# ctu-vras/monoforce

Hardware: AMD Instinct MI355X
Metric: rollout-steps/sec (batch x horizon) on 256x256 terrain (higher is better)
Workload: dtype f32; 1 GPU; c3: B=1024/GPU x T=500 x N=4 contact points, 256x256 grid (res 0.05 m), one shared terrain+friction map (the same on every rank), integrator=odeint-euler (reference default), forward+backward; BASE...; rollouts_per_gpu=1024, rollouts_total=1024, horizon=500, contact_points=4, parallelism=rollout-sharded x1

## Files before the change

monoforce_amd/csrc/physics_loss.hip:

```cpp
#include "mf_common.h"

namespace mf {

__device__ __forceinline__ void atomic_add_s(float* p, float v) { unsafeAtomicAdd(p, v); }
__device__ __forceinline__ void atomic_add_s(double* p, double v) { unsafeAtomicAdd(p, v); }

template <typename S>
__global__ void __launch_bounds__(256) physics_loss_fwd_kernel(const S* __restrict__ Xs, long long sb, long long st,
                                                              const S* __restrict__ Xgt, const S* __restrict__ gt_ts,
                                                              const int* __restrict__ nearest, int B, int T2, S gamma,
                                                              S* __restrict__ partial) {
  __shared__ S wave_sum[4];
  const int i = blockIdx.x * blockDim.x + threadIdx.x;
  S acc = (S)0;
  if (i < B * T2) {
    const int b = i / T2;
    const S w = (S)1 / ((S)1 + gamma * gt_ts[i]);
    const S* x = Xs + b * sb + (long long)nearest[i] * st;
    const S* g = Xgt + (size_t)i * 3;
#pragma unroll
    for (int c = 0; c < 3; ++c) { const S d = x[c] * w - g[c] * w; acc += d * d; }
  }
#pragma unroll
  for (int d = 32; d >= 1; d >>= 1) acc += __shfl_xor(acc, d, 64);
  if ((threadIdx.x & 63) == 0) wave_sum[threadIdx.x >> 6] = acc;
  __syncthreads();
  if (threadIdx.x == 0) partial[blockIdx.x] = (wave_sum[0] + wave_sum[1]) + (wave_sum[2] + wave_sum[3]);
}

template <typename S>
__global__ void __launch_bounds__(256) physics_loss_value_kernel(const S* __restrict__ Xs, long long sb, long long st,
                                                                const S* __restrict__ Xgt, const S* __restrict__ gt_ts,
                                                                const int* __restrict__ nearest, int B, int T2, S gamma,
                                                                S* __restrict__ partial, unsigned* __restrict__ ticket, S inv_count,
                                                                S* __restrict__ loss, S* __restrict__ zero_fill, long long zero_count) {
  __shared__ S wave_sum[4];
  __shared__ bool last;
  const int i = blockIdx.x * blockDim.x + threadIdx.x;
  {
    const long long head = min(zero_count, (long long)(((16u - (unsigned)((uintptr_t)zero_fill & 15u)) & 15u) / sizeof(S)));
    const long long n16 = (zero_count - head) * (long long)sizeof(S) / 16, tail0 = head + n16 * (16 / (long long)sizeof(S));
    int4* z16 = reinterpret_cast<int4*>(zero_fill + head);
    for (long long k = i; k < n16; k += (long long)gridDim.x * blockDim.x) z16[k] = make_int4(0, 0, 0, 0);
    if (i < head) zero_fill[i] = (S)0;
    if (tail0 + i < zero_count) zero_fill[tail0 + i] = (S)0;
  }
  S acc = (S)0;
  if (i < B * T2) {
    const int k = i, b = i / T2;
    const S w = (S)1 / ((S)1 + gamma * gt_ts[k]);
    const S* x = Xs + b * sb + (long long)nearest[k] * st;
    const S* g = Xgt + (size_t)k * 3;
#pragma unroll
    for (int c = 0; c < 3; ++c) { const S d = x[c] * w - g[c] * w; acc += d * d; }
  }
#pragma unroll
  for (int d = 32; d >= 1; d >>= 1) acc += __shfl_xor(acc, d, 64);
  if ((threadIdx.x & 63) == 0) wave_sum[threadIdx.x >> 6] = acc;
  __syncthreads();
  if (threadIdx.x == 0) {
    partial[blockIdx.x] = (wave_sum[0] + wave_sum[1]) + (wave_sum[2] + wave_sum[3]);
    __threadfence();
    last = atomicAdd(ticket, 1u) == gridDim.x - 1;
  }
  __syncthreads();
  if (!last) return;
  __threadfence();
  S tot = (S)0;
  for (unsigned k = threadIdx.x; k < gridDim.x; k += 256) tot += __builtin_nontemporal_load(partial + k);
#pragma unroll
  for (int d = 32; d >= 1; d >>= 1) tot += __shfl_xor(tot, d, 64);
  if ((threadIdx.x & 63) == 0) wave_sum[threadIdx.x >> 6] = tot;
  __syncthreads();
  if (threadIdx.x == 0) {
    loss[0] = ((wave_sum[0] + wave_sum[1]) + (wave_sum[2] + wave_sum[3])) * inv_count;
    *ticket = 0u;
  }
}

template <typename S>
__global__ void __launch_bounds__(256) reduce_grad_copies_kernel(S* __restrict__ pool, int copies, long long n, S* __restrict__ out) {
  const long long i = (long long)blockIdx.x * blockDim.x + threadIdx.x;
  if (i >= n) return;
  S* p = pool + (long long)blockIdx.y * copies * n + i;
  S acc = (S)0;
  for (int c = 0; c < copies; ++c) { acc += p[(long long)c * n]; p[(long long)c * n] = (S)0; }
  out[(long long)blockIdx.y * n + i] = acc;
}

template <typename S>
__global__ void __launch_bounds__(256) physics_loss_bwd_kernel(const S* __restrict__ Xs, long long sb, long long st,
                                                              const S* __restrict__ Xgt, const S* __restrict__ gt_ts,
                                                              const int* __restrict__ nearest, int B, int T2, S gamma,
                                                              const S* __restrict__ gloss, S inv_count, S* __restrict__ gXs) {
  const int t = blockIdx.x * blockDim.x + threadIdx.x;
  if (t >= B * T2) return;
  const bool jm = sb < st;
  const int b = jm ? t % B : t / T2, j = jm ? t / B : t % T2;
  const int i = b * T2 + j;
  const S scale = (S)2 * gloss[0] * inv_count;
  const S w = (S)1 / ((S)1 + gamma * gt_ts[i]);
  const int nr = nearest[i];
  const long long o = b * sb + (long long)nr * st;
  const S* g = Xgt + (size_t)i * 3;
  bool shared = false;
  for (int k = 0; k < T2; ++k) shared |= (k != j) & (nearest[b * T2 + k] == nr);
#pragma unroll
  for (int c = 0; c < 3; ++c) {
    const S v = scale * w * (Xs[o + c] * w - g[c] * w);
    if (shared) atomic_add_s(gXs + o + c, v); else gXs[o + c] = v;
  }
}

template <typename S>
static int loss_fwd(const MfLossDesc* d, const S* Xs, const S* Xgt, const S* gt_ts, const int* nearest, S* partial, hipStream_t st) {
  MF_REQUIRE(d && Xs && Xgt && gt_ts && nearest && partial, MF_ERR_INVALID, "physics_loss_fwd: null argument");
  MF_REQUIRE(d->B > 0 && d->T1 > 0 && d->T2 > 0, MF_ERR_INVALID, "physics_loss_fwd: B, T1, T2 must be positive");
  hipLaunchKernelGGL((physics_loss_fwd_kernel<S>), dim3((d->B * d->T2 + 255) / 256), dim3(256), 0, st, Xs, (long long)d->x_stride_b,
                     (long long)d->x_stride_t, Xgt, gt_ts, nearest, d->B, d->T2, (S)d->gamma, partial);
  hipError_t e = hipGetLastError();
  MF_REQUIRE(e == hipSuccess, MF_ERR_LAUNCH, std::string("physics_loss_fwd launch: ") + hipGetErrorString(e));
  return MF_OK;
}

template <typename S>
static int loss_value(const MfLossDesc* d, const S* Xs, const S* Xgt, const S* gt_ts, const int* nearest, S* partial, unsigned* ticket,
                      S* loss, S* zero_fill, long long zero_count, hipStream_t st) {
  MF_REQUIRE(d && Xs && Xgt && gt_ts && nearest && partial && ticket && loss, MF_ERR_INVALID, "physics_loss_value: null argument");
  MF_REQUIRE(d->B > 0 && d->T1 > 0 && d->T2 > 0, MF_ERR_INVALID, "physics_loss_value: B, T1, T2 must be positive");
  MF_REQUIRE(zero_count >= 0 && (zero_fill || zero_count == 0), MF_ERR_INVALID, "physics_loss_value: zero_count without zero_fill");
  const double count = (double)d->B * d->T2 * 3;
  hipLaunchKernelGGL((physics_loss_value_kernel<S>), dim3((d->B * d->T2 + 255) / 256), dim3(256), 0, st, Xs, (long long)d->x_stride_b,
                     (long long)d->x_stride_t, Xgt, gt_ts, nearest, d->B, d->T2, (S)d->gamma, partial, ticket, (S)(1.0 / count), loss, zero_fill, zero_count);
  hipError_t e = hipGetLastError();
  MF_REQUIRE(e == hipSuccess, MF_ERR_LAUNCH, std::string("physics_loss_value launch: ") + hipGetErrorString(e));
  return MF_OK;
}

template <typename S>
static int reduce_copies(S* pool, int n_maps, int copies, long long n, S* out, hipStream_t st) {
  MF_REQUIRE(pool && out, MF_ERR_INVALID, "reduce_grad_copies: null argument");
  MF_REQUIRE(n_maps > 0 && n_maps < 65536 && copies > 0 && n > 0, MF_ERR_INVALID, "reduce_grad_copies: n_maps, copies, n must be positive");
  hipLaunchKernelGGL((reduce_grad_copies_kernel<S>), dim3((unsigned)((n + 255) / 256), (unsigned)n_maps), dim3(256), 0, st, pool, copies, n, out);
  hipError_t e = hipGetLastError();
  MF_REQUIRE(e == hipSuccess, MF_ERR_LAUNCH, std::string("reduce_grad_copies launch: ") + hipGetErrorString(e));
  return MF_OK;
}

template <typename S>
static int loss_bwd(const MfLossDesc* d, const S* Xs, const S* Xgt, const S* gt_ts, const int* nearest, const S* gloss, S* gXs,
                    hipStream_t st) {
  MF_REQUIRE(d && Xs && Xgt && gt_ts && nearest && gloss && gXs, MF_ERR_INVALID, "physics_loss_bwd: null argument");
  MF_REQUIRE(d->B > 0 && d->T1 > 0 && d->T2 > 0, MF_ERR_INVALID, "physics_loss_bwd: B, T1, T2 must be positive");
  const double count = (double)d->B * d->T2 * 3;
  hipLaunchKernelGGL((physics_loss_bwd_kernel<S>), dim3((d->B * d->T2 + 255) / 256), dim3(256), 0, st, Xs, (long long)d->x_stride_b,
                     (long long)d->x_stride_t, Xgt, gt_ts, nearest, d->B, d->T2, (S)d->gamma, gloss, (S)(1.0 / count), gXs);
  hipError_t e = hipGetLastError();
  MF_REQUIRE(e == hipSuccess, MF_ERR_LAUNCH, std::string("physics_loss_bwd launch: ") + hipGetErrorString(e));
  return MF_OK;
}

}

namespace mf {
template <typename S>
__global__ void __launch_bounds__(256) nearest_steps_kernel(const S* __restrict__ pred_ts, long long pred_sb, const S* __restrict__ gt_ts, long long gt_sb,
                                                           int B, int T1, int T2, int* __restrict__ out) {
  const int i = blockIdx.x * blockDim.x + threadIdx.x;
  if (i >= B * T2) return;
  const int b = i / T2, j = i - b * T2;
  const S g = gt_ts[b * gt_sb + j];
  const S* p = pred_ts + b * pred_sb;
  S best = (S)INFINITY;
  int arg = 0;
  bool any = false;
  int t = 0;
  for (; t + 8 <= T1; t += 8) {
    S v[8];
#pragma unroll
    for (int k = 0; k < 8; ++k) v[k] = p[t + k];
#pragma unroll
    for (int k = 0; k < 8; ++k) {
      const S d = fabs(v[k] - g);
      if (d < best || (!any && d == d)) { best = d; arg = t + k; any = true; }
    }
  }
  for (; t < T1; ++t) {
    const S d = fabs(p[t] - g);
    if (d < best || (!any && d == d)) { best = d; arg = t; any = true; }
  }
  out[i] = arg;
}
template <typename S>
static int nearest_steps(int B, int T1, int T2, const S* pred_ts, long long pred_sb, const S* gt_ts, long long gt_sb, int32_t* out, hipStream_t st) {
  MF_REQUIRE(B > 0 && T1 > 0 && T2 > 0 && pred_ts && gt_ts && out && pred_sb >= 0 && gt_sb >= 0, MF_ERR_INVALID, "nearest_steps: bad argument");
  const long long n = (long long)B * T2;
  MF_REQUIRE(n < (1ll << 31), MF_ERR_UNSUPPORTED, "nearest_steps: B * T2 must be below 2^31");
  hipLaunchKernelGGL((nearest_steps_kernel<S>), dim3((unsigned)((n + 255) / 256)), dim3(256), 0, st, pred_ts, pred_sb, gt_ts, gt_sb, B, T1, T2, out);
  hipError_t e = hipGetLastError();
  MF_REQUIRE(e == hipSuccess, MF_ERR_LAUNCH, std::string("nearest_steps launch: ") + hipGetErrorString(e));
  return MF_OK;
}
}
extern "C" int mf_nearest_steps_f32(int32_t B, int32_t T1, int32_t T2, const float* pred_ts, long long pred_stride_b, const float* gt_ts, long long gt_stride_b,
                                    int32_t* nearest, void* s) { return mf::nearest_steps<float>(B, T1, T2, pred_ts, pred_stride_b, gt_ts, gt_stride_b, nearest, (hipStream_t)s); }
extern "C" int mf_nearest_steps_f64(int32_t B, int32_t T1, int32_t T2, const double* pred_ts, long long pred_stride_b, const double* gt_ts, long long gt_stride_b,
                                    int32_t* nearest, void* s) { return mf::nearest_steps<double>(B, T1, T2, pred_ts, pred_stride_b, gt_ts, gt_stride_b, nearest, (hipStream_t)s); }
extern "C" int mf_physics_loss_fwd_f32(const MfLossDesc* d, const float* Xs, const float* Xgt, const float* gt_ts, const int32_t* nearest,
                                       float* partial, void* s) { return mf::loss_fwd<float>(d, Xs, Xgt, gt_ts, nearest, partial, (hipStream_t)s); }
extern "C" int mf_physics_loss_fwd_f64(const MfLossDesc* d, const double* Xs, const double* Xgt, const double* gt_ts, const int32_t* nearest,
                                       double* partial, void* s) { return mf::loss_fwd<double>(d, Xs, Xgt, gt_ts, nearest, partial, (hipStream_t)s); }
extern "C" int mf_physics_loss_bwd_f32(const MfLossDesc* d, const float* Xs, const float* Xgt, const float* gt_ts, const int32_t* nearest,
                                       const float* gloss, float* gXs, void* s) { return mf::loss_bwd<float>(d, Xs, Xgt, gt_ts, nearest, gloss, gXs, (hipStream_t)s); }
extern "C" int mf_physics_loss_bwd_f64(const MfLossDesc* d, const double* Xs, const double* Xgt, const double* gt_ts, const int32_t* nearest,
                                       const double* gloss, double* gXs, void* s) { return mf::loss_bwd<double>(d, Xs, Xgt, gt_ts, nearest, gloss, gXs, (hipStream_t)s); }
extern "C" int mf_physics_loss_value_f32(const MfLossDesc* d, const float* Xs, const float* Xgt, const float* gt_ts, const int32_t* nearest,
                                         float* partial, uint32_t* ticket, float* loss, float* zero_fill, long long zero_count, void* s) { return mf::loss_value<float>(d, Xs, Xgt, gt_ts, nearest, partial, ticket, loss, zero_fill, zero_count, (hipStream_t)s); }
extern "C" int mf_physics_loss_value_f64(const MfLossDesc* d, const double* Xs, const double* Xgt, const double* gt_ts, const int32_t* nearest,
                                         double* partial, uint32_t* ticket, double* loss, double* zero_fill, long long zero_count, void* s) { return mf::loss_value<double>(d, Xs, Xgt, gt_ts, nearest, partial, ticket, loss, zero_fill, zero_count, (hipStream_t)s); }
extern "C" int mf_reduce_grad_copies_f32(float* pool, int n_maps, int copies, long long n, float* out, void* s) { return mf::reduce_copies<float>(pool, n_maps, copies, n, out, (hipStream_t)s); }
extern "C" int mf_reduce_grad_copies_f64(double* pool, int n_maps, int copies, long long n, double* out, void* s) { return mf::reduce_copies<double>(pool, n_maps, copies, n, out, (hipStream_t)s); }
```

monoforce_amd/csrc/rollout_bwd_cp_kernel.h:

```cpp
#pragma once
#include "rollout_bwd_kernel.h"
#include "rollout_cp_common.h"
#include <type_traits>

namespace mf {

#ifdef MF_STREAM_PROFILE
extern __device__ unsigned long long mf_stream_prof[32];
#define MF_PROF_T(v) const unsigned long long v = __builtin_readcyclecounter()
#define MF_PROF_RT(v) const unsigned long long v = __builtin_amdgcn_s_memrealtime()
#define MF_PROF_ACC(name) unsigned long long name = 0
#define MF_PROF_SUM(name, t0) name += __builtin_readcyclecounter() - (t0)
#define MF_PROF_OUT(slot, val) do { if (lane == 0) atomicAdd(&mf_stream_prof[slot], (unsigned long long)(val)); } while (0)
#define MF_PROF_ADD(slot, t0) MF_PROF_OUT(slot, __builtin_readcyclecounter() - (t0))
#define MF_PROF_MAX(slot, val) do { if (lane == 0) atomicMax(&mf_stream_prof[slot], (unsigned long long)(val)); } while (0)
#define MF_PROF_DRAIN() asm volatile("s_waitcnt vmcnt(0) lgkmcnt(0)" ::: "memory")
#else
#define MF_PROF_T(v)
#define MF_PROF_RT(v)
#define MF_PROF_ACC(name)
#define MF_PROF_SUM(name, t0)
#define MF_PROF_OUT(slot, val)
#define MF_PROF_ADD(slot, t0)
#define MF_PROF_MAX(slot, val)
// ... 928 lines not shown
          const S gzq = -gdh;
          const S dotn = dot3(gn, c.nrm);
          const S gg = (gn - dotn * c.nrm) * c.inlr;
          const S ggp = dpp<0x51>(gg);
          const S nz = mf_fma(gzq, c.wq, cgA * gg + cgB * ggp);
          const S nm = gmuq * c.wq;
          {
            const unsigned ni = (unsigned)c.idx;
            const bool same = !act | (ni == acc_idx);
            st_pending = !same;
            st_idx = acc_idx; st_z = acc_z; st_m = acc_m;
            acc_idx = act ? ni : acc_idx;
            acc_z = same ? acc_z + nz : nz;
            acc_m = same ? acc_m + nm : nm;
          }
          const S vq = gzq * c.zc + gmuq * c.mcv;
          const S gpx = dot4(vq, c.wsb), gpy = dot4(vq, c.wsa);
          const S gp = mask_or(mask_or(mask_or(zero, gpx, lane0), gpy, lane1), gdh, lane2);
          const S gvp1 = dpp<kRot1>(gvp), gvp2 = dpp<kRot2>(gvp);
          gr += gvp1 * c.w2 - gvp2 * c.w1;
          const S gw_p = c.r1 * gvp2 - c.r2 * gvp1;
          const S qa = gp + gr;
          lx += gp; lxd += gvp; lw += gw_p;
          lR0 = mf_fma(qa, P0, lR0); lR1 = mf_fma(qa, P1, lR1); lR2 = mf_fma(qa, P2, lR2);
          S gv = zero, gwc = zero;
          if constexpr (GCTRL) { gv = sum_points(gv_p); gwc = sum_points(gwc_p); }
          lR0 = mf_fma(-dot3(ge_p, c.e), c.eci, mf_fma(ge_p, c.il, lR0));
          gctrl_pending = __builtin_amdgcn_readfirstlane((unsigned)n * kC); gv_pending = gv; gwc_pending = gwc;
        };
        auto crunch = [&](int n, const Coef& c, const UpIn& up, Coef& c_next, UpIn& up_next, auto more, auto paired) {
          add_upstream_masked(up);
          if constexpr (decltype(paired)::value == 1) grab(c_next, up_next);
          else if constexpr (decltype(paired)::value == 2) { grab(c_next, up_next); release(); }
          else if constexpr (decltype(more)::value) take(c_next, up_next);
          flush_stash();
          if constexpr (GCTRL) bstore2(rGctrl, v_ctrl, gctrl_pending, gv_pending, gwc_pending);
#ifdef MF_STREAM_NO_VJP
          asm volatile("" :: "v"(c.R0), "v"(c.w1), "v"(c.f1), "v"(c.NnG), "v"(c.cmdv), "v"(c.csm), "v"(c.dcs), "v"(c.vp), "v"(c.zc), "v"(c.e));
#else
          chain(n, c, up);
#endif
        };
        using std::true_type;
        using std::false_type;
        Coef cA, cB;
        if (n_steps > 0) {
          take(cA, uA);
          MF_PROF_ADD(3, t_k0); MF_PROF_OUT(19, acc_wait);
          using single = std::integral_constant<int, 0>;
          for (; n >= 2; n -= 2) {
            ensure(2);
            crunch(n, cA, uA, cB, uB, true_type{}, std::integral_constant<int, 1>{});
            crunch(n - 1, cB, uB, cA, uA, true_type{}, std::integral_constant<int, 2>{});
          }
          if (n == 1) { crunch(1, cA, uA, cB, uB, true_type{}, single{}); crunch(0, cB, uB, cA, uA, false_type{}, single{}); }
          else crunch(0, cA, uA, cB, uB, false_type{}, single{});
        }
        MF_PROF_ADD(9, t_compute);
        MF_PROF_OUT(8, acc_wait);
#ifdef MF_STREAM_PROFILE
        MF_PROF_OUT(22, acc_wait_early); MF_PROF_OUT(23, n_waited); MF_PROF_OUT(24, acc_wait_late);
#endif
        MF_PROF_ADD(20, t_k0);
        MF_PROF_DRAIN();
        MF_PROF_T(t_sw);
        if (!a.skip_snap) {
          while (__builtin_amdgcn_readfirstlane(vflags[3]) == 0) __builtin_amdgcn_s_sleep(1);
          asm volatile("" ::: "memory");
          snap_idx = idx_of(snap_c[lane]); snap_wq = snap_c[64 + lane]; snap_dx = snap_c[128 + lane]; snap_dy = snap_c[192 + lane];
        }
        MF_PROF_DRAIN();
        MF_PROF_ADD(7, t_sw);
        uA = uZ; uB = uZ;
    } else {
      struct Raw { StateIn st; Saved sv; };
      Raw S_[3];
      Rec K_[3];
      UpIn U_[3];
      auto up_row = [&](int m) { return ODE ? max(m + 1, 0) : max(m, 0); };
      auto run = [&](auto rtag, int n) {
        constexpr int R = decltype(rtag)::value, R1 = (R + 1) % 3, R2 = (R + 2) % 3;
        add_upstream_state(U_[R]);
        gather_cells(S_[R1].sv);
#ifndef MF_SAVED_NO_STATE
        load_state(max(n - 3, 0), S_[R].st);
#endif
#ifndef MF_SAVED_NO_REC
        load_saved(max(n - 3, 0), S_[R].sv);
#endif
#ifndef MF_SAVED_NO_UP
        load_upstream(min(up_row(n - 2), a.T - 1), U_[R2]);
#endif
#ifndef MF_SAVED_NO_ATOMIC
        flush_stash();
#endif
        if constexpr (GCTRL) bstore2(rGctrl, v_ctrl, gctrl_pending, gv_pending, gwc_pending);
#ifndef MF_SAVED_NO_VJP
        vjp(n, K_[R], U_[R]);
#endif
#ifndef MF_SAVED_NO_VJP
        asm("" : "+v"(S_[R1].sv.zc), "+v"(S_[R1].sv.mc) : "v"(lR0));
#endif
#ifndef MF_SAVED_NO_REBUILD
        rebuild(S_[R1].st, S_[R1].sv, K_[R1]);
#endif
      };
      const int n0 = max(n, 0);
      load_state(n0, S_[0].st);
      load_saved(n0, S_[0].sv);
      load_upstream(min(up_row(n0), a.T - 1), U_[0]);
      load_state(max(n0 - 1, 0), S_[1].st);
      load_saved(max(n0 - 1, 0), S_[1].sv);
      load_upstream(min(up_row(n0 - 1), a.T - 1), U_[1]);
      load_state(max(n0 - 2, 0), S_[2].st);
      load_saved(max(n0 - 2, 0), S_[2].sv);
      gather_cells(S_[0].sv);
      rebuild(S_[0].st, S_[0].sv, K_[0]);
      __builtin_amdgcn_s_waitcnt(0);
      using std::integral_constant;
      int i = 0;
      for (; i + 2 < n_steps; i += 3) {
        run(integral_constant<int, 0>{}, n0 - i);
        run(integral_constant<int, 1>{}, n0 - i - 1);
        run(integral_constant<int, 2>{}, n0 - i - 2);
      }
      if (i < n_steps) run(integral_constant<int, 0>{}, n0 - i);
      if (i + 1 < n_steps) run(integral_constant<int, 1>{}, n0 - i - 1);
      {
        const int r0 = (n0 + 1) % 3;
        uA = r0 == 0 ? U_[0] : (r0 == 1 ? U_[1] : U_[2]);
        uB = uA;
      }
      n = -1;
    }
  } else {
  load_state(max(n, 0), sA);
  load_upstream(min(max(n, 0) + (ODE ? 1 : 0), a.T - 1), uA);
  load_state(max(n - 1, 0), sB);
  recompute_gather(sA, recA);
  recompute(recA);
  __builtin_amdgcn_s_waitcnt(0);
  for (; n >= 1; n -= 2) {
    body(n, recA, recB, sB, sA, uA, uB);
    body(n - 1, recB, recA, sA, sB, uB, uA);
  }
  if (n == 0) body(0, recA, recB, sB, sA, uA, uB);
  }
  MF_PROF_T(t_e0);
  UpIn up = (n_steps & 1) ? uB : uA;
  flush_stash();
  if constexpr (GCTRL) bstore2(rGctrl, v_ctrl, gctrl_pending, gv_pending, gwc_pending);
  if (act) emit(acc_idx, acc_z, acc_m);
  if constexpr (ODE) {
    if (n_steps == 0) load_upstream(0, up);
    add_upstream_state(up);
  }
  lx = sum_points(lx); lxd = sum_points(lxd); lw = sum_points(lw);
  lR0 = sum_points(lR0); lR1 = sum_points(lR1); lR2 = sum_points(lR2);
  MF_PROF_DRAIN();
  MF_PROF_ADD(10, t_e0);
  MF_PROF_T(t_s0);

  S gx0 = lx;
  if (!a.skip_snap) {
    if constexpr (!STREAM) snap_cell(snap_idx, snap_wq, snap_dx, snap_dy);
    const S g = dpp<kB2>(lx) / (S)a.N;
    if (act) atomic_add(at32(gzmap, goff + (unsigned)snap_idx), g * snap_wq);
    const S gpx = snap_dx * g * a.inv_res, gpy = snap_dy * g * a.inv_res;
    S gpxy = q == 0 ? gpx : (q == 1 ? gpy : zero);
    gpxy = act ? gpxy : zero;
    gx0 = (q < 2 ? lx : zero) + sum_points(gpxy);
    lR0 += sum_points(gpxy * P0); lR1 += sum_points(gpxy * P1); lR2 += sum_points(gpxy * P2);
  }
  if (p == 0) {
    if (a.gx0) a.gx0[b * 3 + cc] = gx0;
    a.gxd0[b * 3 + cc] = lxd;
    a.gw0[b * 3 + cc] = lw;
    a.gR0[b * 9 + cc * 3 + 0] = lR0; a.gR0[b * 9 + cc * 3 + 1] = lR1; a.gR0[b * 9 + cc * 3 + 2] = lR2;
  }
#ifdef MF_STREAM_PROFILE
  if constexpr (STREAM) {
    MF_PROF_DRAIN();
    MF_PROF_ADD(11, t_s0);
    MF_PROF_RT(rt_end);
    MF_PROF_ADD(12, t_k0);
    MF_PROF_MAX(13, __builtin_readcyclecounter() - t_k0);
    MF_PROF_MAX(14, rt_end); MF_PROF_MAX(15, ~rt_k0); MF_PROF_OUT(16, rt_end - rt_k0);
  }
#endif
  if constexpr (WIN) {
    __syncthreads();
    win_close(a, win, wx0, wy0);
  }
}

int launch_rollout_bwd_cp_f32(const RolloutBwdArgs<float>& a, const BwdRoute& r, int integ, hipStream_t st);
int launch_rollout_bwd_cp_f64(const RolloutBwdArgs<double>& a, const BwdRoute& r, int integ, hipStream_t st);
int launch_rollout_bwd_cp_dynamics_f32(const RolloutBwdArgs<float>& a, const BwdRoute& r, hipStream_t st);
void launch_rollout_bwd_cp_stream_f32(const RolloutBwdArgs<float>& a, const BwdRoute& r, hipStream_t st);
void launch_rollout_bwd_cp_stream_dynamics_f32(const RolloutBwdArgs<float>& a, const BwdRoute& r, hipStream_t st);
void launch_rollout_bwd_cp_stream_f64(const RolloutBwdArgs<double>& a, const BwdRoute& r, hipStream_t st);
inline void launch_rollout_bwd_cp_stream_any(const RolloutBwdArgs<float>& a, int integ, const BwdRoute& r, hipStream_t st) {
  if (integ == MF_INTEG_ODEINT_EULER) launch_rollout_bwd_cp_stream_f32(a, r, st); else launch_rollout_bwd_cp_stream_dynamics_f32(a, r, st);
}
inline void launch_rollout_bwd_cp_stream_any(const RolloutBwdArgs<double>& a, int, const BwdRoute& r, hipStream_t st) {
  launch_rollout_bwd_cp_stream_f64(a, r, st);
}
template <typename S, int INTEG>
int launch_rollout_bwd_cp_variant(const RolloutBwdArgs<S>& a, const BwdRoute& r, hipStream_t st) {
  const unsigned grid = r.grid, block = r.block;
  const int mode = r.cp_mode;
  const bool gc = a.gcontrols != nullptr;
#define MF_BCP(XS_, GC_, M_) MF_KLAUNCH((rollout_bwd_cp_kernel<S, INTEG, XS_, GC_, M_>), dim3(grid), dim3(block), 0, st, a)
  constexpr bool kZmu = std::is_same<S, float>::value && INTEG == MF_INTEG_ODEINT_EULER;
#define MF_BCP_Z(XS_, GC_) do { if constexpr (kZmu) { if (r.zmu) { MF_KLAUNCH((rollout_bwd_cp_kernel<S, INTEG, XS_, GC_, kCpSaved, 6, 3, kZmu>), dim3(grid), dim3(block), 0, st, a); break; } } MF_BCP(XS_, GC_, kCpSaved); } while (0)
  constexpr bool kWin = std::is_same<S, float>::value;
#define MF_BCP_W(XS_, GC_) do { if constexpr (kWin) { if (r.win) { MF_KLAUNCH((rollout_bwd_cp_kernel<S, INTEG, XS_, GC_, kCpEarly, 6, 3, false, kWin>), dim3(grid), dim3(block), 0, st, a); break; } } MF_BCP(XS_, GC_, kCpEarly); } while (0)
#define MF_BCP_L(XS_, GC_) do { if (mode == kCpStream) launch_rollout_bwd_cp_stream_any(a, INTEG, r, st); else if (mode == kCpSaved) MF_BCP_Z(XS_, GC_); else if (mode == kCpLate) MF_BCP(XS_, GC_, kCpLate); else MF_BCP_W(XS_, GC_); } while (0)
  bool one1_done = false;
  if constexpr (std::is_same<S, float>::value) {
    if (r.one1) {
      one1_done = true;
#define MF_BCP1(GC_, W_) MF_KLAUNCH((rollout_bwd_cp_kernel<S, INTEG, true, GC_, kCpEarly, 6, 3, false, W_, true>), dim3(grid), dim3(block), 0, st, a)
#define MF_BCP1_L(GC_) do { if (r.win) MF_BCP1(GC_, kWin); else MF_BCP1(GC_, false); } while (0)
      if (gc) MF_BCP1_L(true); else MF_BCP1_L(false);
#undef MF_BCP1_L
#undef MF_BCP1
    }
  }
  if (!one1_done) {
    if (r.xs_only) { if (gc) MF_BCP_L(true, true); else MF_BCP_L(true, false); }
    else           { if (gc) MF_BCP_L(false, true); else MF_BCP_L(false, false); }
  }
#undef MF_BCP_L
#undef MF_BCP_W
#undef MF_BCP_Z
#undef MF_BCP
  hipError_t e = hipGetLastError();
  MF_REQUIRE(e == hipSuccess, MF_ERR_LAUNCH, std::string("rollout_bwd (component-parallel) launch: ") + hipGetErrorString(e));
  return MF_OK;
}

}
```

monoforce_amd/csrc/rollout_fwd_cp_kernel.h:

```cpp
#pragma once
#include "rollout_cp_common.h"
#include "rollout_fwd_kernel.h"
#include <type_traits>

namespace mf {

template <typename S, int INTEG, bool FORCES, bool ZMU, bool REC, bool LOSS = false>
__global__ void __launch_bounds__(256) __attribute__((amdgpu_waves_per_eu(1, 2))) rollout_fwd_cp_kernel(const RolloutArgs<S> a) {
  using namespace cp;
  using M = Mth<S, std::is_same<S, float>::value>;
  using Msk = typename MaskOf<S>::type;
  constexpr unsigned kS = (unsigned)sizeof(S);
  const int tid = blockIdx.x * blockDim.x + threadIdx.x;
  const int b = (tid >> 4) + a.b0;
  if (b >= a.B) return;
  if (a.loss_poison != nullptr && tid == 0) a.loss_poison[0] = (S)__builtin_nanf("");
  const int p = (tid >> 2) & 3;
  const int q = tid & 3;
  const int cc = q < 3 ? q : 2;
  const S one = S(1.0), zero = S(0.0);
  const int HW = a.H * a.W, last = HW - 1;
  const bool has_mu = a.mu != nullptr;
  const unsigned moff = a.map_shared ? 0u : (unsigned)b * (unsigned)HW;
  const S* zmap = a.z;
  const S* mumap = has_mu ? a.mu : a.z;

  const bool act = p < a.N;
  const int pi = act ? p : 0;
  const S P0 = a.points[pi * 3 + 0], P1 = a.points[pi * 3 + 1], P2 = a.points[pi * 3 + 2];
  const int part = act ? a.part[pi] : -1;
  const S tv_v = part < 0 ? zero : one;
  const S tv_w = part < 0 ? zero : ((part & 1) ? a.half_ly : -a.half_ly);
  const S I0 = a.Iinv[cc * 3 + 0], I1 = a.Iinv[cc * 3 + 1], I2 = a.Iinv[cc * 3 + 2];
  const S grav_c = cc == 2 ? a.mg * a.inv_mass : zero;
  const int cell_off = ((q & 1) ? a.H : 0) + ((q & 2) ? 1 : 0);
  const S wa_s = (q & 2) ? one : -one, wa_o = (q & 2) ? zero : one;
  const S wb_s = (q & 1) ? one : -one, wb_o = (q & 1) ? zero : one;
  const S n_mul = q < 2 ? -a.inv_res : zero, n_add = q < 2 ? zero : one;

  S x, xd, w, R0, R1, R2;
  if (a.default_state) {
    const S v0 = a.controls[(size_t)b * a.ctrl_sb + 0], w0 = a.controls[(size_t)b * a.ctrl_sb + 1];
    x = zero; xd = cc == 0 ? v0 : zero; w = cc == 2 ? w0 : zero;
    R0 = cc == 0 ? one : zero; R1 = cc == 1 ? one : zero; R2 = cc == 2 ? one : zero;
    if (p == 0) {
      S* oxd = const_cast<S*>(a.xd0); S* oR = const_cast<S*>(a.R0); S* ow = const_cast<S*>(a.w0);
      a.x0[b * 3 + cc] = x; oxd[b * 3 + cc] = xd; ow[b * 3 + cc] = w;
      oR[b * 9 + cc * 3 + 0] = R0; oR[b * 9 + cc * 3 + 1] = R1; oR[b * 9 + cc * 3 + 2] = R2;
    }
  } else {
    x = a.x0[b * 3 + cc]; xd = a.xd0[b * 3 + cc]; w = a.w0[b * 3 + cc];
    R0 = a.R0[b * 9 + cc * 3 + 0]; R1 = a.R0[b * 9 + cc * 3 + 1]; R2 = a.R0[b * 9 + cc * 3 + 2];
  }

  auto footprint = [&](S pc, int* idx, S* wq, S* ou = nullptr) {
    const S lim = S(262144.0);
    const S u = M::cell_coord(pc, a.d_max, a.res, a.inv_res);
    const int ui = (int)M::clamp(u, -lim, lim);
    const S fr = u - (S)ui;
    const int base = dppi<kB1>(ui) + __mul24(a.H, dppi<kB0>(ui));
    *idx = min(max(base + cell_off, 0), last);
    const S wa = mf_fma(wa_s, dpp<kB0>(fr), wa_o), wb = mf_fma(wb_s, dpp<kB1>(fr), wb_o);
    *wq = wa * wb;
    if (ou) *ou = u;
  };

  if (!a.skip_snap) {
    const S pc = (P0 * R0 + P1 * R1 + P2 * R2) + x;
    int idx; S wq;
    footprint(pc, &idx, &wq);
    const S zq = dot4(wq, ld32(zmap, moff + (unsigned)idx));
    const S acc = sum_points(act ? zq : zero);
    const S xz = acc / (S)a.N;
    x = cc == 2 ? xz : x;
    if (p == 0 && q == 2) a.x0[b * 3 + 2] = xz;
  }

  const unsigned row_stride = (a.layout == MF_LAYOUT_TIME_MAJOR) ? (unsigned)a.B : 1u;
  const unsigned row0 = (a.layout == MF_LAYOUT_TIME_MAJOR) ? (unsigned)b : (unsigned)b * (unsigned)a.T;
  S* v3base = p == 0 ? a.Xs : p == 1 ? a.Xds : p == 2 ? a.Om : (a.Xraw ? a.Xraw : a.Xs);
  const S sink_l = (p == 3 && a.Xraw) ? zero : a.sink;
  const Msk m_xd = p == 1 ? ~(Msk)0 : (Msk)0, m_w = p == 2 ? ~(Msk)0 : (Msk)0, m_x = ~(m_xd | m_w);
  char* p3 = reinterpret_cast<char*>(v3base) + (size_t)(row0 * 3u + (unsigned)cc) * kS;
  const Rsrc rCtrl = make_rsrc(a.controls);
  unsigned o9 = (row0 * 9u + (unsigned)cc * 3u) * kS;
  const unsigned frow = (unsigned)a.fstride * 3u;
  unsigned ofs = (row0 * frow + (unsigned)p * 3u + (unsigned)cc) * kS, off = ofs;
  const unsigned d3 = row_stride * 3u * kS, d9 = row_stride * 9u * kS, df = row_stride * frow * kS;
  const char* pRs = reinterpret_cast<const char*>(a.Rs);
  const char* pFs = reinterpret_cast<const char*>(a.Fs);
  const char* pFf = reinterpret_cast<const char*>(a.Ff);

  S oFs = zero, oFf = zero;

  auto emit_row = [&](S ex, S exd, S ew, S e0, S e1, S e2, unsigned adv) {
    const S vx = mf_fma(e2, sink_l, ex);
    const S v3 = mask_or(mask_or(mask_or(zero, vx, m_x), exd, m_xd), ew, m_w);
    __builtin_nontemporal_store(v3, reinterpret_cast<S*>(p3));
    bstore3(pRs, o9, 0u, e0, e1, e2);
    if (FORCES) { bstore1(pFs, ofs, 0u, oFs); bstore1(pFf, off, 0u, oFf); }
    if (adv) { p3 += d3; o9 += d9; ofs += df; off += df; }
  };

  const int n_steps = (INTEG == MF_INTEG_ODEINT_EULER) ? a.T - 1 : a.T;
  unsigned v_ctrl = (unsigned)b * (unsigned)a.ctrl_sb * kS;
  S cv, cw;
  bload2(rCtrl, v_ctrl, 0u, &cv, &cw);
  S h_ode = (INTEG == MF_INTEG_ODEINT_EULER && a.T > 1) ? a.ts[1] - a.ts[0] : zero;
  struct Geo { S r, pc, wq, zc, mc, e, u, il, coln2; int idx; };
  auto geometry = [&](S gx, S g0, S g1, S g2) {
    Geo g;
    g.r = cp_body_r(P0, P1, P2, g0, g1, g2);
    g.pc = g.r + gx;
    footprint(g.pc, &g.idx, &g.wq, &g.u);
    const int idx = g.idx;
    if constexpr (ZMU) {
      const Pk2<S> zm = *reinterpret_cast<const Pk2<S>*>(reinterpret_cast<const char*>(a.zmu) + (size_t)((unsigned)idx * 2u * kS));
      g.zc = zm.a; g.mc = zm.b;
    } else {
      g.zc = ld32(zmap, moff + (unsigned)idx);
      g.mc = ld32(mumap, moff + (unsigned)idx);
    }
    g.coln2 = dot3(g0, g0);
    g.il = M::inv_len(g.coln2);
    g.e = g0 * g.il;
    return g;
  };
  char* const pRec0 = reinterpret_cast<char*>(a.rec);
  unsigned rec_off = (unsigned)tid * kRecBytesPerLane<S>;
  const unsigned rec_step = (unsigned)a.B * 16u * kRecBytesPerLane<S>;
  typedef S f4v __attribute__((ext_vector_type(4)));
  auto rec_store = [&](const f4v& rq, unsigned adv) {
#if defined(MF_REC_NOSTORE)
    asm volatile("" :: "v"(rq));
#elif defined(MF_REC_PLAIN)
    *reinterpret_cast<f4v*>(pRec0 + (size_t)rec_off) = rq;
#else
    __builtin_nontemporal_store(rq, reinterpret_cast<f4v*>(pRec0 + (size_t)rec_off));
#endif
    if (adv) rec_off += rec_step;
  };
  auto contact = [&](const Geo& g, S vxd, S vw, S tv, S* xdd, S* wd, S* oFr, S* oFf, f4v* rq) {
    const S vp = cp_vel(vxd, vw, g.r);
    const S zq = dot4(g.wq, g.zc);
    const S mub = dot4(g.wq, has_mu ? g.mc : one);
    const S dz = g.zc - dpp<kB0>(g.zc);
    const S u = mf_fma(dpp<kN12>(dz), n_mul, n_add);
    const S inl = M::inv_len(dot3(u, u));
    const S nrm = u * inl;
    const S dh = dpp<kB2>(g.pc) - zq;
    S cj = M::sigmoid_m10(dh);
    cj = act ? cj : zero;
    const S csum = sum_points(cj);
    const S inv_csum = M::div(one, csum);
    const S vn = dot3(vp, nrm);
    const S A = cp_normal_force(a.k, dh, a.damp, vn);
    const S Fr = M::clamp(cp_spring(A, nrm, cj, inv_csum), -a.mg, a.mg);
    const S Nn = M::sqrt(dot3(Fr, Fr));
    const S s = mub * cp_cmd(tv, g.e, vp);
    const S sn = dot3(s, nrm);
    const S Ff = M::clamp(Nn * cp_tangent(s, sn, nrm), -a.mg, a.mg);
    const S f = Fr + Ff;
    const S tau = unrot(cross_pre(g.r, f));
    const S Fsum = sum_points(f), Tsum = sum_points(tau);
    const S wraw = cp_wraw(I0, I1, I2, Tsum);
    *wd = M::clamp(wraw, -a.omega_max, a.omega_max);
    *xdd = Fsum * a.inv_mass - grav_c;
    *oFr = Fr; *oFf = Ff;
    if constexpr (REC) *rq = f4v{g.u, cj, wraw, A};
  };

  S l_acc = zero;
  int l_j = 0;
  const int l_last = LOSS ? a.loss_T2 - 1 : 0;
  const unsigned l_lane = LOSS ? ((unsigned)b * (unsigned)a.loss_T2 * 3u + (unsigned)cc) : 0u;
  struct Stamp { S g, w; };
  auto loss_peek = [&](int row) {
    Stamp st = {zero, zero};
    if constexpr (LOSS) {
      st.g = ld32(a.loss_gt, l_lane + (unsigned)(min(l_j, l_last) * 3));
      st.w = a.loss_row_w[row];
    }
    return st;
  };
  auto loss_row = [&](S ex, S e2, const Stamp& st) {
    if constexpr (LOSS) {
      const S term = cp_loss_term(mf_fma(e2, a.sink, ex), st.g, st.w);
      l_acc += st.w != zero ? term : zero;
      l_j += st.w != zero ? 1 : 0;
    }
  };

  if constexpr (INTEG == MF_INTEG_ODEINT_EULER) {
    S t_cur = a.T > 1 ? a.ts[1] : zero;
    const unsigned ctrl_step = (unsigned)a.ctrl_st * kS, v_ctrl_last = v_ctrl + (unsigned)(a.T - 1) * ctrl_step;
    auto ode_step = [&](int n, const Geo& g, Geo& g_next, S cv_n, S cw_n, S h, S& cv_next, S& cw_next, S& h_next) {
      v_ctrl = min(v_ctrl + ctrl_step, v_ctrl_last);
      bload2(rCtrl, v_ctrl, 0u, &cv_next, &cw_next);
      const S t_next = a.ts[min(n + 2, a.T - 1)];
      const Stamp stamp = loss_peek(n + 1);
      const S tv = cp_track(tv_v, tv_w, cv_n, cw_n);
      const S d0 = h * cross_pre(w, R0), d1 = h * cross_pre(w, R1), d2 = h * cross_pre(w, R2);
      const S xn = mf_fma(h, xd, x);
      const S Rn0 = R0 + unrot(d0), Rn1 = R1 + unrot(d1), Rn2 = R2 + unrot(d2);
      g_next = geometry(xn, Rn0, Rn1, Rn2);
      emit_row(x, xd, w, R0, R1, R2, 1u);
      x = xn; R0 = Rn0; R1 = Rn1; R2 = Rn2;
      S xdd, wd, Fr, Ff;
      f4v rq;
      contact(g, xd, w, tv, &xdd, &wd, &Fr, &Ff, &rq);
      if constexpr (REC) rec_store(rq, 1u);
      xd = mf_fma(h, xdd, xd);
      w = mf_fma(h, wd, w);
      oFs = mf_fma(h, Fr, oFs);
      oFf = mf_fma(h, Ff, oFf);
      h_next = t_next - t_cur;
      t_cur = t_next;
      loss_row(x, R2, stamp);
    };
    Geo gA, gB;
    S cvA = cv, cwA = cw, hA = h_ode, cvB = zero, cwB = zero, hB = zero;
    if (n_steps > 0) gA = geometry(x, R0, R1, R2);
    loss_row(x, R2, loss_peek(0));
    __builtin_amdgcn_s_waitcnt(0);
    int n = 0;
    for (; n + 1 < n_steps; n += 2) {
      ode_step(n, gA, gB, cvA, cwA, hA, cvB, cwB, hB);
      ode_step(n + 1, gB, gA, cvB, cwB, hB, cvA, cwA, hA);
    }
    if (n < n_steps) ode_step(n, gA, gB, cvA, cwA, hA, cvB, cwB, hB);
  } else {
    __builtin_amdgcn_s_waitcnt(0);
    for (int n = 0; n < n_steps; ++n) {
      const int nn = min(n + 1, a.T - 1);
      S cv_next, cw_next;
      bload2(rCtrl, v_ctrl, __builtin_amdgcn_readfirstlane((unsigned)(nn * a.ctrl_st) * kS), &cv_next, &cw_next);
      const S tv = cp_track(tv_v, tv_w, cv, cw);
      S xdd, wd, Fr, Ff;
      const Geo g = geometry(x, R0, R1, R2);
      emit_row(x, xd, w, R0, R1, R2, n > 0 ? 1u : 0u);
      f4v rq;
      contact(g, xd, w, tv, &xdd, &wd, &Fr, &Ff, &rq);
      if constexpr (REC) rec_store(rq, 1u);
      const S h = a.dt;
      xd = mf_fma(xdd, h, xd);
      x = mf_fma(xd, h, x);
      w = mf_fma(wd, h, w);
      const S th2 = dot3(w, w);
      const S il = M::inv_len(th2);
      const S kc = w * il;
      const S k1 = dpp<kRot1>(kc), k2 = dpp<kRot2>(kc);
      S sn_, oc;
      M::sincos_small(M::len_of(th2, il) * h, &sn_, &oc);
      const S kk = M::kReciprocalNorm ? th2 * (il * il) : dot3(kc, kc);
      const S ock = oc * kc;
      const S m0 = one + oc * (kc * kc - kk);
      const S m1 = mf_fma(ock, k1, -(sn_ * k2));
      const S m2 = mf_fma(ock, k2, sn_ * k1);
      const S n0 = R0 * dpp<kB0>(m0) + R1 * dpp<kB1>(m2) + R2 * dpp<kB2>(m1);
      const S n1 = R0 * dpp<kB0>(m1) + R1 * dpp<kB1>(m0) + R2 * dpp<kB2>(m2);
      const S n2 = R0 * dpp<kB0>(m2) + R1 * dpp<kB1>(m1) + R2 * dpp<kB2>(m0);
      R0 = n0; R1 = n1; R2 = n2;
      oFs = Fr; oFf = Ff;
      cv = cv_next; cw = cw_next;
    }
  }
  if (n_steps > 0 || INTEG == MF_INTEG_ODEINT_EULER) emit_row(x, xd, w, R0, R1, R2, 1u);
  if constexpr (LOSS) {
    static_assert(!LOSS || INTEG == MF_INTEG_ODEINT_EULER, "the fused loss rides on the default integrator's kernels");
    __shared__ S l_sh[80];
    const int lane = threadIdx.x;
    if (lane < 16) l_sh[lane] = zero;
    if (p == 0 && q < 3) l_sh[(lane >> 4) * 4 + q] = l_acc;
    __syncthreads();
    unsigned last = 0u;
    if (lane == 0) {
      S tot = zero;
#pragma unroll
      for (int r = 0; r < 4; ++r) tot += (l_sh[r * 4 + 0] + l_sh[r * 4 + 1]) + l_sh[r * 4 + 2];
      __builtin_nontemporal_store(tot, a.loss_partial + blockIdx.x);
      __threadfence();
      last = atomicAdd(a.loss_ticket, 1u) == gridDim.x - 1 ? 1u : 0u;
    }
    last = __builtin_amdgcn_readfirstlane(last);
    if (last) {
      __threadfence();
      const int n_act = min(64, (a.B - (int)blockIdx.x * 4) * 16);
      S tot = zero;
      for (unsigned k2 = (unsigned)lane; k2 < gridDim.x; k2 += (unsigned)n_act) tot += __builtin_nontemporal_load(a.loss_partial + k2);
      l_sh[16 + lane] = tot;
      __syncthreads();
      if (lane == 0) {
        S sum = zero;
        for (int k2 = 0; k2 < n_act; ++k2) sum += l_sh[16 + k2];
        a.loss_out[0] = sum * a.loss_inv_count;
        *a.loss_ticket = 0u;
      }
    }
  }
}

int launch_rollout_fwd_cp_f32(const RolloutArgs<float>& a, const FwdRoute& r, int integ, hipStream_t st);
int launch_rollout_fwd_cp_f64(const RolloutArgs<double>& a, const FwdRoute& r, int integ, hipStream_t st);
template <typename S>
int launch_rollout_fwd_cp_t(const RolloutArgs<S>& a, const FwdRoute& r, int integ, hipStream_t st) {
  const int block = r.block;
  const unsigned grid = (unsigned)(((long long)a.B * 16 + block - 1) / block);
  const bool forces = r.forces, zmu = r.zmu;
  const bool rec = r.record;
  if (r.loss == kLossInLaunch) {
    constexpr int I = MF_INTEG_ODEINT_EULER;
    if (rec) { if (zmu) MF_KLAUNCH((rollout_fwd_cp_kernel<S, I, false, true, true, true>), dim3(grid), dim3(block), 0, st, a);
               else MF_KLAUNCH((rollout_fwd_cp_kernel<S, I, false, false, true, true>), dim3(grid), dim3(block), 0, st, a); }
    else     { if (zmu) MF_KLAUNCH((rollout_fwd_cp_kernel<S, I, false, true, false, true>), dim3(grid), dim3(block), 0, st, a);
               else MF_KLAUNCH((rollout_fwd_cp_kernel<S, I, false, false, false, true>), dim3(grid), dim3(block), 0, st, a); }
    hipError_t e = hipGetLastError();
    MF_REQUIRE(e == hipSuccess, MF_ERR_LAUNCH, std::string("rollout_fwd (component-parallel, fused loss) launch: ") + hipGetErrorString(e));
    return MF_OK;
  }
#define MF_CP(INTEG_, FORCES_, ZMU_) do { if (rec) MF_KLAUNCH((rollout_fwd_cp_kernel<S, INTEG_, FORCES_, ZMU_, true>), dim3(grid), dim3(block), 0, st, a); \
                                          else MF_KLAUNCH((rollout_fwd_cp_kernel<S, INTEG_, FORCES_, ZMU_, false>), dim3(grid), dim3(block), 0, st, a); } while (0)
#define MF_CP_F(INTEG_)                                          \
  do {                                                           \
    if (forces) { if (zmu) MF_CP(INTEG_, true, true); else MF_CP(INTEG_, true, false); }    \
    else        { if (zmu) MF_CP(INTEG_, false, true); else MF_CP(INTEG_, false, false); }  \
  } while (0)
  if (integ == MF_INTEG_DYNAMICS) MF_CP_F(MF_INTEG_DYNAMICS); else MF_CP_F(MF_INTEG_ODEINT_EULER);
#undef MF_CP_F
#undef MF_CP
  hipError_t e = hipGetLastError();
  MF_REQUIRE(e == hipSuccess, MF_ERR_LAUNCH, std::string("rollout_fwd (component-parallel) launch: ") + hipGetErrorString(e));
  return MF_OK;
}


}
```

Before: 1.384 billion rollout-steps/s.

## Vectorize grad-copy reduction and trim forward ODE slot/time loads

The gradient-copy reduction kernel now uses 16-byte vector loads, a 16-deep unrolled batch of loads across copies, a grid-stride loop with 64-thread blocks, and skips writing zeros back to slots that are already zero. The forward ODE kernel replaces mask-based component selection with a plain select, loads timestamps through a buffer resource with a running offset instead of indexed global loads, and simplifies the paired-loop bound. The backward kernel avoids a redundant upstream load in streaming mode when there are no steps. These aim to cut memory traffic and VGPR/ALU work, at the cost of extra code paths and a data-dependent store branch in the reduction.

Result: faster. 1.439 billion rollout-steps/s (median of 6 runs) (+3.9%).

```diff
diff --git a/monoforce_amd/csrc/physics_loss.hip b/monoforce_amd/csrc/physics_loss.hip
--- a/monoforce_amd/csrc/physics_loss.hip
+++ b/monoforce_amd/csrc/physics_loss.hip
@@ -78,8 +78,9 @@
   }
 }
 
-template <typename S>
-__global__ void __launch_bounds__(256) reduce_grad_copies_kernel(S* __restrict__ pool, int copies, long long n, S* __restrict__ out) {
+#if defined(MF_REDUCE_OLD)
+template <typename S>
+__global__ void __launch_bounds__(256) reduce_grad_copies_kernel(S* __restrict__ pool, int copies, long long n, S* __restrict__ out, int) {
   const long long i = (long long)blockIdx.x * blockDim.x + threadIdx.x;
   if (i >= n) return;
   S* p = pool + (long long)blockIdx.y * copies * n + i;
@@ -87,6 +88,60 @@
   for (int c = 0; c < copies; ++c) { acc += p[(long long)c * n]; p[(long long)c * n] = (S)0; }
   out[(long long)blockIdx.y * n + i] = acc;
 }
+constexpr int kReduceThreads = 256;
+#else
+constexpr int kReduceUnroll = 16;
+constexpr int kReduceThreads = 64;
+template <typename S, int W> struct ReduceVec { typedef S type __attribute__((ext_vector_type(W))); };
+template <typename S> struct ReduceVec<S, 1> { typedef S type; };
+template <typename V>
+__device__ __forceinline__ bool any_bit(const V& v) {
+  if constexpr (sizeof(V) == 16) {
+    typedef unsigned u4v __attribute__((ext_vector_type(4)));
+    const u4v u = __builtin_bit_cast(u4v, v);
+    return ((u.x | u.y) | (u.z | u.w)) != 0u;
+  } else if constexpr (sizeof(V) == 8) {
+    return __builtin_bit_cast(unsigned long long, v) != 0ull;
+  } else {
+    return __builtin_bit_cast(unsigned, v) != 0u;
+  }
+}
+template <typename S, int W>
+__device__ __forceinline__ void reduce_grad_copies_body(S* __restrict__ pool, int copies, long long n, S* __restrict__ out) {
+  typedef typename ReduceVec<S, W>::type V;
+  constexpr int K = kReduceUnroll;
+  const long long items = n / W;
+  S* const map = pool + (long long)blockIdx.y * copies * n;
+  S* const o = out + (long long)blockIdx.y * n;
+  for (long long i = (long long)blockIdx.x * blockDim.x + threadIdx.x; i < items; i += (long long)gridDim.x * blockDim.x) {
+    V* const p = reinterpret_cast<V*>(map + i * W);
+    const long long sc = n / W;
+    V acc = V{};
+    int c = 0;
+    for (; c + K <= copies; c += K) {
+      V v[K];
+#pragma unroll
+      for (int k = 0; k < K; ++k) v[k] = p[(long long)(c + k) * sc];
+#pragma unroll
+      for (int k = 0; k < K; ++k) {
+        acc += v[k];
+        if (any_bit(v[k])) p[(long long)(c + k) * sc] = V{};
+      }
+    }
+    for (; c < copies; ++c) {
+      const V v = p[(long long)c * sc];
+      acc += v;
+      if (any_bit(v)) p[(long long)c * sc] = V{};
+    }
+    *reinterpret_cast<V*>(o + i * W) = acc;
+  }
+}
+template <typename S>
+__global__ void __launch_bounds__(kReduceThreads) reduce_grad_copies_kernel(S* __restrict__ pool, int copies, long long n, S* __restrict__ out, int wide) {
+  if (wide) reduce_grad_copies_body<S, 16 / (int)sizeof(S)>(pool, copies, n, out);
+  else reduce_grad_copies_body<S, 1>(pool, copies, n, out);
+}
+#endif
 
 template <typename S>
 __global__ void __launch_bounds__(256) physics_loss_bwd_kernel(const S* __restrict__ Xs, long long sb, long long st,
@@ -141,7 +196,15 @@
 static int reduce_copies(S* pool, int n_maps, int copies, long long n, S* out, hipStream_t st) {
   MF_REQUIRE(pool && out, MF_ERR_INVALID, "reduce_grad_copies: null argument");
   MF_REQUIRE(n_maps > 0 && n_maps < 65536 && copies > 0 && n > 0, MF_ERR_INVALID, "reduce_grad_copies: n_maps, copies, n must be positive");
-  hipLaunchKernelGGL((reduce_grad_copies_kernel<S>), dim3((unsigned)((n + 255) / 256), (unsigned)n_maps), dim3(256), 0, st, pool, copies, n, out);
+  constexpr long long kW = 16 / (long long)sizeof(S);
+#if defined(MF_REDUCE_OLD)
+  const int wide = 0;
+#else
+  const int wide = ((uintptr_t)pool % 16 == 0 && (uintptr_t)out % 16 == 0 && n % kW == 0) ? 1 : 0;
+#endif
+  const long long items = wide ? n / kW : n;
+  const long long blocks = std::min((items + kReduceThreads - 1) / kReduceThreads, 1ll << 20);
+  hipLaunchKernelGGL((reduce_grad_copies_kernel<S>), dim3((unsigned)blocks, (unsigned)n_maps), dim3(kReduceThreads), 0, st, pool, copies, n, out, wide);
   hipError_t e = hipGetLastError();
   MF_REQUIRE(e == hipSuccess, MF_ERR_LAUNCH, std::string("reduce_grad_copies launch: ") + hipGetErrorString(e));
   return MF_OK;
diff --git a/monoforce_amd/csrc/rollout_bwd_cp_kernel.h b/monoforce_amd/csrc/rollout_bwd_cp_kernel.h
--- a/monoforce_amd/csrc/rollout_bwd_cp_kernel.h
+++ b/monoforce_amd/csrc/rollout_bwd_cp_kernel.h
@@ -1104,7 +1104,7 @@
   if constexpr (GCTRL) bstore2(rGctrl, v_ctrl, gctrl_pending, gv_pending, gwc_pending);
   if (act) emit(acc_idx, acc_z, acc_m);
   if constexpr (ODE) {
-    if (n_steps == 0) load_upstream(0, up);
+    if (n_steps == 0 && !STREAM) load_upstream(0, up);
     add_upstream_state(up);
   }
   lx = sum_points(lx); lxd = sum_points(lxd); lw = sum_points(lw);
diff --git a/monoforce_amd/csrc/rollout_fwd_cp_kernel.h b/monoforce_amd/csrc/rollout_fwd_cp_kernel.h
--- a/monoforce_amd/csrc/rollout_fwd_cp_kernel.h
+++ b/monoforce_amd/csrc/rollout_fwd_cp_kernel.h
@@ -9,7 +9,6 @@
 __global__ void __launch_bounds__(256) __attribute__((amdgpu_waves_per_eu(1, 2))) rollout_fwd_cp_kernel(const RolloutArgs<S> a) {
   using namespace cp;
   using M = Mth<S, std::is_same<S, float>::value>;
-  using Msk = typename MaskOf<S>::type;
   constexpr unsigned kS = (unsigned)sizeof(S);
   const int tid = blockIdx.x * blockDim.x + threadIdx.x;
   const int b = (tid >> 4) + a.b0;
@@ -80,7 +79,12 @@
   const unsigned row0 = (a.layout == MF_LAYOUT_TIME_MAJOR) ? (unsigned)b : (unsigned)b * (unsigned)a.T;
   S* v3base = p == 0 ? a.Xs : p == 1 ? a.Xds : p == 2 ? a.Om : (a.Xraw ? a.Xraw : a.Xs);
   const S sink_l = (p == 3 && a.Xraw) ? zero : a.sink;
+#if defined(MF_FWD_SLOTS_OLD)
+  using Msk = typename MaskOf<S>::type;
   const Msk m_xd = p == 1 ? ~(Msk)0 : (Msk)0, m_w = p == 2 ? ~(Msk)0 : (Msk)0, m_x = ~(m_xd | m_w);
+#else
+  const bool is_xd = p == 1, is_w = p == 2;
+#endif
   char* p3 = reinterpret_cast<char*>(v3base) + (size_t)(row0 * 3u + (unsigned)cc) * kS;
   const Rsrc rCtrl = make_rsrc(a.controls);
   unsigned o9 = (row0 * 9u + (unsigned)cc * 3u) * kS;
@@ -95,7 +99,11 @@
 
   auto emit_row = [&](S ex, S exd, S ew, S e0, S e1, S e2, unsigned adv) {
     const S vx = mf_fma(e2, sink_l, ex);
+#if defined(MF_FWD_SLOTS_OLD)
     const S v3 = mask_or(mask_or(mask_or(zero, vx, m_x), exd, m_xd), ew, m_w);
+#else
+    const S v3 = is_xd ? exd : is_w ? ew : vx;
+#endif
     __builtin_nontemporal_store(v3, reinterpret_cast<S*>(p3));
     bstore3(pRs, o9, 0u, e0, e1, e2);
     if (FORCES) { bstore1(pFs, ofs, 0u, oFs); bstore1(pFf, off, 0u, oFf); }
@@ -194,10 +202,21 @@
   if constexpr (INTEG == MF_INTEG_ODEINT_EULER) {
     S t_cur = a.T > 1 ? a.ts[1] : zero;
     const unsigned ctrl_step = (unsigned)a.ctrl_st * kS, v_ctrl_last = v_ctrl + (unsigned)(a.T - 1) * ctrl_step;
+#if !defined(MF_FWD_SLOTS_OLD)
+    const Rsrc rTs = make_rsrc(a.ts);
+    unsigned v_ts = kS;
+    const unsigned v_ts_last = (unsigned)(a.T - 1) * kS;
+    asm volatile("" : "+v"(v_ts));
+#endif
     auto ode_step = [&](int n, const Geo& g, Geo& g_next, S cv_n, S cw_n, S h, S& cv_next, S& cw_next, S& h_next) {
       v_ctrl = min(v_ctrl + ctrl_step, v_ctrl_last);
       bload2(rCtrl, v_ctrl, 0u, &cv_next, &cw_next);
+#if defined(MF_FWD_SLOTS_OLD)
       const S t_next = a.ts[min(n + 2, a.T - 1)];
+#else
+      v_ts = min(v_ts + kS, v_ts_last);
+      const S t_next = bload1<S>(rTs, v_ts, 0u);
+#endif
       const Stamp stamp = loss_peek(n + 1);
       const S tv = cp_track(tv_v, tv_w, cv_n, cw_n);
       const S d0 = h * cross_pre(w, R0), d1 = h * cross_pre(w, R1), d2 = h * cross_pre(w, R2);
@@ -224,7 +243,12 @@
     loss_row(x, R2, loss_peek(0));
     __builtin_amdgcn_s_waitcnt(0);
     int n = 0;
-    for (; n + 1 < n_steps; n += 2) {
+#if defined(MF_FWD_SLOTS_OLD)
+    const int n_pairs = n_steps - 1;
+#else
+    const int n_pairs = n_steps & ~1;
+#endif
+    for (; n < n_pairs; n += 2) {
       ode_step(n, gA, gB, cvA, cwA, hA, cvB, cwB, hB);
       ode_step(n + 1, gB, gA, cvB, cwB, hB, cvA, cwA, hA);
     }
```
